# dendisuhubdy/neural_sound_generation

Hardware: AMD Instinct MI355X
Metric: mel-frames/sec VQ-VAE fwd+bwd+Adam (80-mel x 1024) (higher is better)
Workload: dtype bf16; 1 GPU; BASELINE configs[1]: VQVAE(1,dim=128,z_dim=512) train step, 128 clips/GPU x 80-mel x 1024 frames; clips_per_gpu=128, global_batch=128, frames=1024, parallelism=dp1

## Files before the change

### include/nsg.h

```cpp
#ifndef NSG_H_
#define NSG_H_

#include <stdint.h>
#include <stddef.h>

#ifdef __cplusplus
extern "C" {
#endif

#if defined(__GNUC__)
#define NSG_API __attribute__((visibility("default")))
#else
#define NSG_API
#endif

#define NSG_VERSION 104

enum {
    NSG_OK = 0,
    NSG_E_INVALID = -1,
    NSG_E_UNSUPPORTED = -2,
    NSG_E_WORKSPACE = -3
};

// ... 126 lines not shown
                            size_t workspace_bytes, void *stream);

NSG_API size_t nsg_c1conv_bn_workspace_bytes(int32_t C);
NSG_API int nsg_c1conv_bn_relu_forward(const float *img, const float *w, const float *bias, const float *gamma, const float *beta,
                                       float *mean, float *invstd, float *running_mean, float *running_var, float eps,
                                       float momentum, int32_t training, void *y, int32_t y_dtype, int32_t B, int32_t H,
                                       int32_t W, int32_t C, void *workspace, size_t workspace_bytes, double *moments,
                                       void *stream);
NSG_API int nsg_c1conv_bn_relu_backward(const float *img, const float *w, const float *bias, const float *gamma,
                                        const float *beta, const float *mean, const float *invstd, const void *dy,
                                        int32_t dy_dtype, float *dw, float *dbias, float *dgamma, float *dbeta, int32_t B,
                                        int32_t H, int32_t W, int32_t C, void *workspace, size_t workspace_bytes,
                                        const double *moments, void *stream);
#define NSG_C1_MOMENTS 273

NSG_API int32_t nsg_bn_relu_c1convt_supported(int32_t dtype, int32_t C);
NSG_API size_t nsg_bn_relu_c1convt_workspace_bytes(int32_t B, int32_t H, int32_t W, int32_t C);
NSG_API int nsg_bn_relu_c1convt_forward(const void *u, int32_t dtype, const float *mean, const float *invstd, const float *gamma,
                                        const float *beta, const float *w, const float *bias, float *y, int32_t flags, int32_t B,
                                        int32_t H, int32_t W, int32_t C, void *workspace, size_t workspace_bytes, void *stream);
NSG_API int nsg_bn_relu_c1convt_forward_mse(const void *u, int32_t dtype, const float *mean, const float *invstd, const float *gamma,
                                            const float *beta, const float *w, const float *bias, float *y, const float *target,
                                            int32_t T, float grad_scale, float *loss_out, float *dpre, float *dbias, int32_t B,
                                            int32_t H, int32_t W, int32_t C, void *workspace, size_t workspace_bytes, void *stream);
NSG_API int nsg_bn_relu_c1convt_backward(const void *u, int32_t dtype, const float *mean, const float *invstd, const float *gamma,
                                         const float *beta, const float *w, const float *dy, void *du, float *du_colsum, float *dw,
                                         float *dbias, float *dgamma, float *dbeta, int32_t B, int32_t H, int32_t W, int32_t C,
                                         void *workspace, size_t workspace_bytes, void *stream);

NSG_API int32_t nsg_bn_relu_conv1x1_supported(int32_t dtype, int32_t C);
// ... 239 lines not shown
```

### neural_sound_generation_amd/_lib.py

```python
from __future__ import annotations

import ctypes
import os
import re
from ctypes import POINTER, Structure, c_char_p, c_float, c_int32, c_int64, c_size_t, c_void_p

from .build import INCLUDE

_PKG = os.path.dirname(os.path.abspath(__file__))
LIB_PATH = os.path.join(_PKG, "libnsg.so")
HEADER_PATH = os.path.join(INCLUDE, "nsg.h")


class NsgError(RuntimeError):
    pass


class ConvDesc(Structure):

    def key(self):
        return tuple(getattr(self, f) for f, _ in self._fields_)


_SCALARS = {"int": c_int32, "int32_t": c_int32, "int64_t": c_int64, "size_t": c_size_t, "float": c_float}
# ... 50 lines not shown
            return parse_header(f.read())
    except OSError as e:
        raise NsgError(f"{HEADER_PATH}: cannot read the ABI header ({e})")


_SIGS, _CONSTS, _fields = _header()
if not _fields:
    raise NsgError(f"{HEADER_PATH}: struct nsg_conv_desc not found")
ConvDesc._fields_ = [(f, c_int32) for f in _fields]
HEADER_SYMBOLS = list(_SIGS)
NSG_VERSION = _CONSTS["NSG_VERSION"]
NSG_RELU_IN, NSG_TANH_OUT, NSG_OUT_F32, NSG_RELU_OUT, NSG_F32, NSG_BF16, NSG_C1_MOMENTS = (_CONSTS[n] for n in (
    "NSG_RELU_IN", "NSG_TANH_OUT", "NSG_OUT_F32", "NSG_RELU_OUT", "NSG_F32", "NSG_BF16", "NSG_C1_MOMENTS"))
NSG_DTW_MAX_FRAMES, NSG_DTW_BLOCK_COLS = _CONSTS["NSG_DTW_MAX_FRAMES"], _CONSTS["NSG_DTW_BLOCK_COLS"]
NSG_F0_MAX_CANDIDATES, NSG_F0_VITERBI_LDS_FRAMES = _CONSTS["NSG_F0_MAX_CANDIDATES"], _CONSTS["NSG_F0_VITERBI_LDS_FRAMES"]

_lib = None


def _bind(lib):
    for name, (res, args) in _SIGS.items():
        fn = getattr(lib, name)
        fn.argtypes = args
        fn.restype = res
    if lib.nsg_version() != NSG_VERSION:
        raise NsgError(f"the HIP library reports ABI version {lib.nsg_version()}, include/nsg.h declares version {NSG_VERSION}: rebuild it "
                       "(python -m neural_sound_generation_amd.build --force)")
    return lib


DIAG_LIB_PATH = os.path.join(_PKG, "libnsg_diag.so")
_DIAG_SWITCHES = {"nsg_debug_set_patch_gemm": c_int32, "nsg_debug_set_patch_grid": c_int32, "nsg_debug_set_wgrad_strip": c_int32,
                  "nsg_debug_set_c1_moments": c_int32, "nsg_debug_set_wgrad_bf16_native": c_int32, "nsg_debug_set_wgrad_stagger": c_int32,
                  "nsg_debug_set_wgrad_diag": c_int32, "nsg_debug_set_wgrad_stamp_buffer": c_void_p, "nsg_debug_set_stamp_buffer": c_void_p,
                  "nsg_debug_set_f0_direct": c_int32}
_diag = None


def load_diag():
    global _diag
    if _diag is None:
        import torch
        if not os.path.exists(DIAG_LIB_PATH):
            raise NsgError(f"{DIAG_LIB_PATH} is missing: python -m neural_sound_generation_amd.build --diag")
        lib = _bind(ctypes.CDLL(DIAG_LIB_PATH))
        for name, at in _DIAG_SWITCHES.items():
            fn = getattr(lib, name)
            fn.argtypes = [at]
            fn.restype = None
        _diag = lib
# ... 60 lines not shown
```

### neural_sound_generation_amd/csrc/c1_mfma.hip

```cpp
#include "nsg_reduce.h"
#include "c1_geom.h"
#include <type_traits>

namespace {

typedef float v2f __attribute__((ext_vector_type(2)));

template <int NT> struct PatchRegs { static constexpr int N = (PATCH_VALS + NT - 1) / NT; };

template <int NT>
__device__ __forceinline__ void patch_load(float (&r)[PatchRegs<NT>::N], const float *__restrict__ img, const C1Geom &g, int b, int ly, int ox0, int tid)
{
    constexpr int NCOL = 2 * TW + 2;
#pragma unroll
    for (int q = 0; q < PatchRegs<NT>::N; ++q) {
        const int i = tid + NT * q;
        const int rr = i / NCOL, cix = i - rr * NCOL;
        const int y = 2 * ly - 1 + rr, x = 2 * ox0 - 1 + cix;
        const bool ok = (i < PATCH_VALS) & (y >= 0) & (y < g.HH) & (x >= 0) & (x < g.WW);
        const float v = img[ok ? ((size_t)b * g.HH + y) * g.WW + x : 0];
        r[q] = ok ? v : 0.f;
    }
}
template <int NT>
// ... 738 lines not shown
    }
    const double bs = b + sft * wsum;
    const double Sp = mom[mom_sum(t)];
    const double St = Sp + (double)M * sft;
    const double X = is * (pw + (bs - mu) * Sp);
    const double G = (double)dw[e];
    dw[e] = (float)(sc * (G - (double)dbeta[c] * inv * St - (double)dgamma[c] * inv * X));
    if (t == 0 && dbias) {
        double sh = (double)M * bs;
#pragma unroll
        for (int u = 0; u < 16; ++u) sh += (double)w[(size_t)c * 16 + u] * mom[mom_sum(u)];
        dbias[c] = (float)(-sc * (double)dgamma[c] * inv * is * (sh - (double)M * mu));
    }
}

template <int NW>
__global__ __launch_bounds__(256) void bnrelu_dots_kernel(const bf16_t *__restrict__ u, const float *__restrict__ mean,
                                                          const float *__restrict__ invstd, const float *__restrict__ gamma,
                                                          const float *__restrict__ beta, const float *__restrict__ w,
                                                          float *__restrict__ dots, int64_t M)
{
    constexpr int C = 32 * NW, KS = C / 16, ROWS = 128, CPR = C / 8, PIECES = ROWS * CPR / 256;
    __shared__ __attribute__((aligned(16))) bf16_t tile[ROWS * gpitch(C)];
    __shared__ __attribute__((aligned(16))) float cfs[C], coff[C];
    const int tid = threadIdx.x, lane = tid & 63, wave = tid >> 6;
    const int n = lane & 31, hb = lane >> 5;
    for (int c = tid; c < C; c += 256) {
        const float fs = invstd[c] * gamma[c];
        cfs[c] = fs;
        coff[c] = __builtin_fmaf(-mean[c], fs, beta[c]);
    }
    v4u wa[KS];
#pragma unroll
    for (int ks = 0; ks < KS; ++ks)
#pragma unroll
        for (int i = 0; i < 4; ++i) {
            const int c0 = 16 * ks + 8 * hb + 2 * i;
            const unsigned pk = pack_bf16(w[(size_t)c0 * 16 + (n & 15)], w[(size_t)(c0 + 1) * 16 + (n & 15)]);
            wa[ks][i] = n < 16 ? pk : 0u;
        }
    const int64_t ntiles = (M + ROWS - 1) / ROWS;
    v4f pr[PIECES];
    auto prefetch = [&](int64_t t) {
#pragma unroll
        for (int i = 0; i < PIECES; ++i) {
            const int q = tid + 256 * i;
            const int row = q / CPR, cc = q - row * CPR;
            const int64_t m = t * ROWS + row;
            pr[i] = *reinterpret_cast<const v4f *>(u + (size_t)(m < M ? m : M - 1) * C + 8 * cc);
        }
    };
    auto stage = [&]() {
#pragma unroll
        for (int i = 0; i < PIECES; ++i) {
            const int q = tid + 256 * i;
            const int row = q / CPR, cc = q - row * CPR;
            *reinterpret_cast<v4f *>(tile + row * gpitch(C) + 8 * cc) = pr[i];
        }
    };
    if ((int64_t)blockIdx.x < ntiles) { prefetch(blockIdx.x); stage(); }
    __syncthreads();
    for (int64_t t = blockIdx.x; t < ntiles; t += gridDim.x) {
        const int64_t nxt = t + gridDim.x;
        if (nxt < ntiles) prefetch(nxt);
        v16f acc;
#pragma unroll
        for (int r = 0; r < 16; ++r) acc[r] = 0.f;
        const bf16_t *rowp = tile + (32 * wave + n) * gpitch(C) + 8 * hb;
#pragma unroll
        for (int ks = 0; ks < KS; ++ks) {
            const v4f raw = *reinterpret_cast<const v4f *>(rowp + 16 * ks);
            const v4f f0 = *reinterpret_cast<const v4f *>(cfs + 16 * ks + 8 * hb), f1 = *reinterpret_cast<const v4f *>(cfs + 16 * ks + 8 * hb + 4);
            const v4f o0 = *reinterpret_cast<const v4f *>(coff + 16 * ks + 8 * hb), o1 = *reinterpret_cast<const v4f *>(coff + 16 * ks + 8 * hb + 4);
            const float fs8[8] = {f0.x, f0.y, f0.z, f0.w, f1.x, f1.y, f1.z, f1.w};
            const float of8[8] = {o0.x, o0.y, o0.z, o0.w, o1.x, o1.y, o1.z, o1.w};
            float uv[8];
            Elem<bf16_t>::unpack16(raw, uv);
            v4u a;
#pragma unroll
            for (int i = 0; i < 4; ++i)
                a[i] = pack_bf16(fmaxf(__builtin_fmaf(uv[2 * i], fs8[2 * i], of8[2 * i]), 0.f),
                                 fmaxf(__builtin_fmaf(uv[2 * i + 1], fs8[2 * i + 1], of8[2 * i + 1]), 0.f));
            acc = __builtin_amdgcn_mfma_f32_32x32x16_bf16(__builtin_bit_cast(bf16x8, wa[ks]), __builtin_bit_cast(bf16x8, a), acc, 0, 0, 0);
        }
        const int64_t m = t * ROWS + 32 * wave + n;
        if (m < M) {
            *reinterpret_cast<v4f *>(dots + (size_t)m * 16 + 4 * hb) = v4f{acc[0], acc[1], acc[2], acc[3]};
            *reinterpret_cast<v4f *>(dots + (size_t)m * 16 + 8 + 4 * hb) = v4f{acc[4], acc[5], acc[6], acc[7]};
        }
        __syncthreads();
        if (nxt < ntiles) stage();
        __syncthreads();
    }
}

}

bool nsg_c1m_supported(int C) { return (C % 32 == 0 && C >= 32 && C <= 128) || C == 256; }

#define NSG_C1M_DISPATCH(KERNEL, ...)                                                                                   \
    switch (C / 32) {                                                                                                   \
    case 1: hipLaunchKernelGGL((KERNEL<1>), dim3(blocks), dim3(64), 0, s, __VA_ARGS__); break;                          \
    case 2: hipLaunchKernelGGL((KERNEL<2>), dim3(blocks), dim3(128), 0, s, __VA_ARGS__); break;                         \
    case 3: hipLaunchKernelGGL((KERNEL<3>), dim3(blocks), dim3(192), 0, s, __VA_ARGS__); break;                         \
    case 8: hipLaunchKernelGGL((KERNEL<8>), dim3(blocks), dim3(512), 0, s, __VA_ARGS__); break;                         \
    default: hipLaunchKernelGGL((KERNEL<4>), dim3(blocks), dim3(256), 0, s, __VA_ARGS__); break;                        \
    }
// ... 98 lines not shown
    int64_t blocks = (M + 127) / 128;
    const int64_t cap = C > 128 ? 512 : 1024;
    if (blocks > cap) blocks = cap;
    if (blocks < 1) return NSG_OK;
    const bf16_t *ub = reinterpret_cast<const bf16_t *>(u);
    switch (C / 32) {
    case 1: hipLaunchKernelGGL((bnrelu_dots_kernel<1>), dim3((unsigned)blocks), dim3(256), 0, s, ub, mean, invstd, gamma, beta, w, dots, M); break;
    case 2: hipLaunchKernelGGL((bnrelu_dots_kernel<2>), dim3((unsigned)blocks), dim3(256), 0, s, ub, mean, invstd, gamma, beta, w, dots, M); break;
    case 3: hipLaunchKernelGGL((bnrelu_dots_kernel<3>), dim3((unsigned)blocks), dim3(256), 0, s, ub, mean, invstd, gamma, beta, w, dots, M); break;
    case 8: hipLaunchKernelGGL((bnrelu_dots_kernel<8>), dim3((unsigned)blocks), dim3(256), 0, s, ub, mean, invstd, gamma, beta, w, dots, M); break;
    default: hipLaunchKernelGGL((bnrelu_dots_kernel<4>), dim3((unsigned)blocks), dim3(256), 0, s, ub, mean, invstd, gamma, beta, w, dots, M); break;
    }
    return nsg_check_launch("bnrelu_dots_kernel");
}

int nsg_launch_c1m_out_bwd_sums(const float *dimg, const float *w, const void *u, const float *mean, const float *invstd, const float *gamma,
                                const float *beta, float *partial, int blocks, int B, int LH, int LW, int C, hipStream_t s)
{
    const C1Geom g = make_geom(B, LH, LW, 2 * LH, 2 * LW, C);
    NSG_C1M_DISPATCH2(c1m_bwd_sums_kernel, true, dimg, w, (const float *)nullptr, reinterpret_cast<const bf16_t *>(u), mean, invstd, gamma, beta,
                      partial, g)
    return nsg_check_launch("c1m_bwd_sums_kernel<out>");
}

int nsg_launch_c1m_out_bwd_apply(const float *dimg, const float *w, const void *u, const float *mean, const float *invstd, const float *gamma,
                                 const float *beta, const float *dgamma, const float *dbeta, float inv_m, float *partial17, void *du, int blocks,
                                 int B, int LH, int LW, int C, hipStream_t s)
{
    const C1Geom g = make_geom(B, LH, LW, 2 * LH, 2 * LW, C);
    NSG_C1M_DISPATCH2(c1m_bwd_wgrad_kernel, true, dimg, w, (const float *)nullptr, reinterpret_cast<const bf16_t *>(u), mean, invstd, gamma, beta,
// ... 4 lines not shown
```

### neural_sound_generation_amd/csrc/conv_api.hip

```cpp
#include "nsg_reduce.h"

NSG_DIAG_SWITCH(unsigned long long *, g_debug_stamps, nullptr)
#ifdef NSG_DIAG
extern "C" NSG_API void nsg_debug_set_stamp_buffer(unsigned long long *buf) { g_debug_stamps = buf; }
#endif

namespace {

struct PackJob {
    const float *src;
    void *dst;
    int T, NN, CC, sn, sc, flip, bf16, frag;
};
constexpr int PACK_MAX_JOBS = 32;
struct PackJobs {
    PackJob job[PACK_MAX_JOBS];
};
__global__ __launch_bounds__(256) void pack_w_kernel(const PackJobs jobs)
{
    const PackJob j = jobs.job[blockIdx.y];
    const int64_t total = (int64_t)j.T * j.NN * j.CC;
    if (j.bf16 && j.CC % 8 == 0 && (reinterpret_cast<uintptr_t>(j.dst) & 15u) == 0) {
        typedef unsigned u4 __attribute__((ext_vector_type(4)));
        const int CG = j.CC / 8;
// ... 25 lines not shown
                reinterpret_cast<bf16_t *>(j.dst)[total + nsg_frag_index(t, n, c, j.NN, j.CC)] = nsg_f2bf(v);
            }
        } else {
            reinterpret_cast<float *>(j.dst)[i] = v;
        }
    }
}

constexpr int C1_COL2IM_TY = 4, C1_COL2IM_TX = 64;
inline int col2im_blocks(int B, int HH, int WW)
{
    const int64_t nt = (int64_t)B * (((HH + 1) / 2 + C1_COL2IM_TY - 1) / C1_COL2IM_TY) * (((WW + 1) / 2 + C1_COL2IM_TX - 1) / C1_COL2IM_TX);
    return (int)(nt < C1_LOSS_BLOCKS ? (nt < 1 ? 1 : nt) : C1_LOSS_BLOCKS);
}

__device__ __forceinline__ float c1_tanh(float x)
{
    const float t = __expf(-2.f * fabsf(x));
    return copysignf(__fdividef(1.f - t, 1.f + t), x);
}
constexpr int C2I_TY = C1_COL2IM_TY, C2I_TX = C1_COL2IM_TX;
static_assert(C2I_TY * C2I_TX == 256, "one thread per position");
template <bool LOSS>
__global__ __launch_bounds__(256) void col2im_c1_kernel(const float *__restrict__ dots, const float *__restrict__ bias, float *__restrict__ out,
                                                        int B, int LH, int LW, int HH, int WW, int tanh_out, const float *__restrict__ target,
                                                        int T, float gscale, float *__restrict__ dpre, double *__restrict__ partial)
{
    typedef float f2 __attribute__((ext_vector_type(2)));
    constexpr int RY = C2I_TY + 2, RX = C2I_TX + 2, RP = 16 + 4;
    __shared__ __attribute__((aligned(16))) float rec[RY * RX * RP];
    const int PY = (HH + 1) / 2, PX = (WW + 1) / 2;
    const int tiles_y = (PY + C2I_TY - 1) / C2I_TY, tiles_x = (PX + C2I_TX - 1) / C2I_TX;
    const int64_t ntiles = (int64_t)B * tiles_y * tiles_x;
    const int tid = threadIdx.x;
    const int py = tid / C2I_TX, px = tid - py * C2I_TX;
    const float bv = bias ? bias[0] : 0.f;
    const bool vec = (T & 1) == 0, vec_out = (WW & 1) == 0;
    double lacc = 0.0, gacc = 0.0;
    constexpr int NPC = (RY * RX * 4 + 255) / 256;
    v4f pc[NPC];
    auto tile_coords = [&](int64_t tile, int &b, int &ly0, int &lx0) {
        const int tx = (int)(tile % tiles_x);
        const int ty = (int)((tile / tiles_x) % tiles_y);
// ... 31 lines not shown
        if (ly >= PY || lx >= PX) continue;
        const float *rc = rec + ((py + 1) * RX + (px + 1)) * RP;
        auto tap = [&](int m, int n, int kh, int kw) { return rc[((m - 1) * RX + (n - 1)) * RP + 4 * kh + kw]; };
        float o[2][2];
        o[0][0] = (((bv + tap(1, 1, 1, 1)) + tap(1, 0, 1, 3)) + tap(0, 1, 3, 1)) + tap(0, 0, 3, 3);
        o[0][1] = (((bv + tap(1, 2, 1, 0)) + tap(1, 1, 1, 2)) + tap(0, 2, 3, 0)) + tap(0, 1, 3, 2);
        o[1][0] = (((bv + tap(2, 1, 0, 1)) + tap(2, 0, 0, 3)) + tap(1, 1, 2, 1)) + tap(1, 0, 2, 3);
        o[1][1] = (((bv + tap(2, 2, 0, 0)) + tap(2, 1, 0, 2)) + tap(1, 2, 2, 0)) + tap(1, 1, 2, 2);
        float l4 = 0.f, g4 = 0.f;
#pragma unroll
        for (int j = 0; j < 2; ++j) {
            const int yo = 2 * ly + j, xo = 2 * lx;
            if (yo >= HH) continue;
            const bool two = xo + 1 < WW;
            const size_t io = ((size_t)b * HH + yo) * WW + xo;
            const float v0 = tanh_out ? c1_tanh(o[j][0]) : o[j][0], v1 = tanh_out ? c1_tanh(o[j][1]) : o[j][1];
            if (out) {
                if (vec_out) *reinterpret_cast<f2 *>(out + io) = f2{v0, v1};
                else { out[io] = v0; if (two) out[io + 1] = v1; }
            }
            if (LOSS) {
                const float *tp = target + ((size_t)b * HH + yo) * T + xo;
                f2 tv;
                if (vec) tv = *reinterpret_cast<const f2 *>(tp);
                else { tv.x = tp[0]; tv.y = two ? tp[1] : 0.f; }
                const float d0 = v0 - tv.x, d1 = two ? v1 - tv.y : 0.f;
                l4 = __builtin_fmaf(d1, d1, __builtin_fmaf(d0, d0, l4));
                const float gp0 = gscale * d0 * (1.f - v0 * v0), gp1 = two ? gscale * d1 * (1.f - v1 * v1) : 0.f;
                if (vec_out) *reinterpret_cast<f2 *>(dpre + io) = f2{gp0, gp1};
                else { dpre[io] = gp0; if (two) dpre[io + 1] = gp1; }
                g4 += gp0;
                g4 += gp1;
                if (lx == PX - 1)
                    for (int xx = WW; xx < T; ++xx) {
                        const float cv = target[((size_t)b * HH + yo) * T + xx];
                        lacc += (double)(cv * cv);
                    }
            }
        }
        lacc += (double)l4;
        gacc += (double)g4;
    }
    if (LOSS) {
        nsg_block_sum_four_walk(lacc, partial);
        __syncthreads();
        nsg_block_sum_four_walk(gacc, partial + gridDim.x);
    }
}

constexpr int CS_MAX_SLABS = 512;
template <typename TI>
__global__ __launch_bounds__(256) void colsum_partial_kernel(const TI *__restrict__ x, int64_t M, int C, int slab_rows,
                                                             float *__restrict__ partial)
{
    __shared__ float red[256];
    const int tid = threadIdx.x;
    const int Cb = C < 256 ? C : 256;
    const int rgroups = 256 / Cb;
    const int cl = tid % Cb, rg = tid / Cb;
    const int64_t r0 = (int64_t)blockIdx.x * slab_rows;
    const int64_t r1 = min(M, r0 + slab_rows);
    for (int cb = 0; cb < C; cb += Cb) {
// ... 492 lines not shown

int nsg_bn_relu_c1convt_forward(const void *u, int32_t dtype, const float *mean, const float *invstd, const float *gamma, const float *beta,
                                const float *w, const float *bias, float *y, int32_t flags, int32_t B, int32_t H, int32_t W, int32_t C,
                                void *workspace, size_t workspace_bytes, void *stream)
{
    NSG_REQUIRE(u && mean && invstd && gamma && beta && w && y, NSG_E_INVALID, "nsg_bn_relu_c1convt_forward: null pointer");
    NSG_REQUIRE(B > 0 && H > 0 && W > 0, NSG_E_INVALID, "nsg_bn_relu_c1convt_forward: bad extent");
    NSG_REQUIRE(nsg_bn_relu_c1convt_supported(dtype, C), NSG_E_UNSUPPORTED,
                "nsg_bn_relu_c1convt_forward: needs bf16 tensors and C = 32, 64, 96 or 128 (use the separate operators otherwise)");
    NSG_REQUIRE(!(flags & ~NSG_TANH_OUT), NSG_E_UNSUPPORTED, "nsg_bn_relu_c1convt_forward: only NSG_TANH_OUT");
    NSG_REQUIRE(nsg_aligned16(u) && nsg_aligned16(w), NSG_E_INVALID, "nsg_bn_relu_c1convt_forward: u and w must be 16-byte aligned");
    NSG_REQUIRE(workspace && workspace_bytes >= nsg_bn_relu_c1convt_workspace_bytes(B, H, W, C), NSG_E_WORKSPACE,
                "nsg_bn_relu_c1convt_forward: workspace too small");
    NSG_REQUIRE((int64_t)B * H * W * C <= 0x7fffffffLL * 4, NSG_E_UNSUPPORTED, "nsg_bn_relu_c1convt_forward: tensor too large");
    hipStream_t s = (hipStream_t)stream;
    float *dots = c1t_fwd_layout(workspace, B, H, W).dots;
    int rc = nsg_launch_bnrelu_dots(u, mean, invstd, gamma, beta, w, dots, (int64_t)B * H * W, C, s);
    if (rc) return rc;
    hipLaunchKernelGGL(col2im_c1_kernel<false>, dim3(col2im_blocks(B, 2 * H, 2 * W)), dim3(256), 0, s, dots, bias, y, B, H, W, 2 * H,
                       2 * W, (flags & NSG_TANH_OUT) ? 1 : 0, (const float *)nullptr, 0, 0.f, (float *)nullptr, (double *)nullptr);
    return nsg_check_launch("col2im_c1_kernel");
}

int nsg_bn_relu_c1convt_forward_mse(const void *u, int32_t dtype, const float *mean, const float *invstd, const float *gamma, const float *beta,
                                    const float *w, const float *bias, float *y, const float *target, int32_t T, float grad_scale,
                                    float *loss_out, float *dpre, float *dbias, int32_t B, int32_t H, int32_t W, int32_t C, void *workspace,
                                    size_t workspace_bytes, void *stream)
{
    NSG_REQUIRE(u && mean && invstd && gamma && beta && w && target && loss_out && dpre, NSG_E_INVALID, "nsg_bn_relu_c1convt_forward_mse: null pointer");
    NSG_REQUIRE(B > 0 && H > 0 && W > 0 && T >= 2 * W, NSG_E_INVALID, "nsg_bn_relu_c1convt_forward_mse: bad extent (T >= 2W)");
    NSG_REQUIRE(nsg_bn_relu_c1convt_supported(dtype, C), NSG_E_UNSUPPORTED,
                "nsg_bn_relu_c1convt_forward_mse: needs bf16 tensors and C = 32, 64, 96, 128 or 256 (use the separate operators otherwise)");
    NSG_REQUIRE(nsg_aligned16(u) && nsg_aligned16(w), NSG_E_INVALID, "nsg_bn_relu_c1convt_forward_mse: u and w must be 16-byte aligned");
    NSG_REQUIRE(workspace && workspace_bytes >= nsg_bn_relu_c1convt_workspace_bytes(B, H, W, C), NSG_E_WORKSPACE,
                "nsg_bn_relu_c1convt_forward_mse: workspace too small");
    NSG_REQUIRE((int64_t)B * H * W * C <= 0x7fffffffLL * 4, NSG_E_UNSUPPORTED, "nsg_bn_relu_c1convt_forward_mse: tensor too large");
    hipStream_t s = (hipStream_t)stream;
    const C1tFwdLayout L = c1t_fwd_layout(workspace, B, H, W);
    float *dots = L.dots;
    double *partial = L.partial;
    int rc = nsg_launch_bnrelu_dots(u, mean, invstd, gamma, beta, w, dots, (int64_t)B * H * W, C, s);
    if (rc) return rc;
    const int64_t n = (int64_t)B * 2 * H * T;
    const int nb = col2im_blocks(B, 2 * H, 2 * W);
    hipLaunchKernelGGL(col2im_c1_kernel<true>, dim3(nb), dim3(256), 0, s, dots, bias, y, B, H, W, 2 * H, 2 * W, 1, target, T,
                       grad_scale * 2.0f / (float)n, dpre, partial);
    rc = nsg_check_launch("col2im_c1_kernel<loss>");
    if (rc) return rc;
    rc = nsg_launch_final_mean(partial, nb, (double)n, loss_out, s);
    if (rc || !dbias) return rc;
    return nsg_launch_final_mean(partial + nb, nb, 1.0, dbias, s);
}

int nsg_bn_relu_c1convt_backward(const void *u, int32_t dtype, const float *mean, const float *invstd, const float *gamma, const float *beta,
                                 const float *w, const float *dy, void *du, float *du_colsum, float *dw, float *dbias, float *dgamma,
                                 float *dbeta, int32_t B, int32_t H, int32_t W, int32_t C, void *workspace, size_t workspace_bytes,
                                 void *stream)
{
    NSG_REQUIRE(u && mean && invstd && gamma && beta && w && dy && du && dw && dgamma && dbeta, NSG_E_INVALID,
                "nsg_bn_relu_c1convt_backward: null pointer");
    NSG_REQUIRE(B > 0 && H > 0 && W > 0, NSG_E_INVALID, "nsg_bn_relu_c1convt_backward: bad extent");
    NSG_REQUIRE(nsg_bn_relu_c1convt_supported(dtype, C), NSG_E_UNSUPPORTED,
                "nsg_bn_relu_c1convt_backward: needs bf16 tensors and C = 32, 64, 96 or 128 (use the separate operators otherwise)");
    NSG_REQUIRE(nsg_aligned16(u) && nsg_aligned16(du) && nsg_aligned16(w), NSG_E_INVALID, "nsg_bn_relu_c1convt_backward: u, du and w must be 16-byte aligned");
    NSG_REQUIRE(workspace && workspace_bytes >= nsg_bn_relu_c1convt_workspace_bytes(B, H, W, C), NSG_E_WORKSPACE,
                "nsg_bn_relu_c1convt_backward: workspace too small");
// ... 146 lines not shown
```

### neural_sound_generation_amd/csrc/nsg_common.h

```cpp
#pragma once
#include <hip/hip_runtime.h>
#include <stdint.h>
#include <stdio.h>
#include <stdarg.h>
#include <atomic>
#include <initializer_list>
#include "nsg.h"

typedef float v4f __attribute__((ext_vector_type(4)));
typedef float v16f __attribute__((ext_vector_type(16)));
typedef short s16x8 __attribute__((ext_vector_type(8)));
typedef short s16x4 __attribute__((ext_vector_type(4)));
typedef __bf16 bf16x8 __attribute__((ext_vector_type(8)));
typedef unsigned short bf16_t;

__host__ __device__ __forceinline__ unsigned nsg_fbits(float f) { return __builtin_bit_cast(unsigned, f); }
__host__ __device__ __forceinline__ float nsg_bitsf(unsigned u) { return __builtin_bit_cast(float, u); }

__device__ __forceinline__ bf16_t nsg_f2bf(float f) { return __builtin_bit_cast(bf16_t, (__bf16)f); }
typedef float nsg_v2f __attribute__((ext_vector_type(2)));
typedef __bf16 nsg_bf16x2 __attribute__((ext_vector_type(2)));
__device__ __forceinline__ unsigned nsg_pack_bf16(float a, float b)
{
    const nsg_v2f f = {a, b};
// ... 213 lines not shown
int nsg_launch_flat1x1_backward(const void *h, const void *dy, const float *mean, const float *invstd, const float *gamma, const float *dgamma,
                                const float *dbeta, const float *w, void *dh, void *dx, int64_t M, int C, void *ws, int *nblocks,
                                const void *prev_x, const float *prev_mean, const float *prev_invstd, const float *prev_gamma,
                                const float *prev_beta, float **prev_partial, hipStream_t s);
bool nsg_flat1x1_fused_bwd_supported(int dtype, int C);
size_t nsg_flat1x1_fused_bwd_workspace_bytes(int C);
int nsg_launch_flat1x1_fused_bwd(const void *h, const void *dy, const float *mean, const float *invstd, const float *gamma, const float *dgamma,
                                 const float *dbeta, const float *w, void *dx, float *dw, int64_t M, int C, void *ws, int *nblocks,
                                 const void *prev_x, const float *prev_mean, const float *prev_invstd, const float *prev_gamma,
                                 const float *prev_beta, float **colsum_partial, float **prev_partial, float **dw_partial, hipStream_t s);
int nsg_launch_final_mean(const double *partial, int n, double denom, float *out, hipStream_t s);
constexpr int C1_LOSS_BLOCKS = 1024;
bool nsg_c1m_supported(int C);
int nsg_launch_bnrelu_dots(const void *u, const float *mean, const float *invstd, const float *gamma, const float *beta, const float *w,
                           float *dots, int64_t M, int C, hipStream_t s);
int nsg_launch_c1m_out_bwd_sums(const float *dimg, const float *w, const void *u, const float *mean, const float *invstd, const float *gamma,
                                const float *beta, float *partial, int blocks, int B, int LH, int LW, int C, hipStream_t s);
int nsg_launch_c1m_out_bwd_apply(const float *dimg, const float *w, const void *u, const float *mean, const float *invstd, const float *gamma,
                                 const float *beta, const float *dgamma, const float *dbeta, float inv_m, float *partial17, void *du, int blocks,
                                 int B, int LH, int LW, int C, hipStream_t s);
int nsg_launch_c1m_stats(const float *img, const float *w, const float *bias, float *tiles, int blocks, int B, int LH, int LW, int HH, int WW,
                         int C, hipStream_t s);
int nsg_launch_c1m_apply(const float *img, const float *w, const float *bias, const float *mean, const float *invstd, const float *gamma,
                         const float *beta, void *out, int blocks, int B, int LH, int LW, int HH, int WW, int C, hipStream_t s);
int nsg_launch_c1m_bwd_sums(const float *img, const float *w, const float *bias, const void *dy, const float *mean, const float *invstd,
                            const float *gamma, const float *beta, float *partial, int blocks, int B, int LH, int LW, int HH, int WW, int C,
                            hipStream_t s);
int nsg_launch_c1m_bwd_wgrad(const float *img, const float *w, const float *bias, const void *dy, const float *mean, const float *invstd,
                             const float *gamma, const float *beta, const float *dgamma, const float *dbeta, float inv_m, float *partial,
                             int blocks, int B, int LH, int LW, int HH, int WW, int C, hipStream_t s);
// ... 15 lines not shown
```

Measured before the change: 16.82 million mel-frames/s.

## Fuse BN-ReLU dots and col2im into banded transposed-conv kernel

Adds a banded kernel for the final transposed conv that computes the BN+ReLU 1x1 dot products with MFMA per row band and resolves the col2im overlap in shared memory. It emits tanh output, the MSE loss and dpre directly, so the intermediate dots tensor no longer makes a round trip through global memory. The two final-mean launches are also merged into one two-block kernel. In exchange the new kernel has halo recomputation, more synchronisation per row, and a more complex loss and boundary path.

New measurement: 16.92 million mel-frames/s, median of 6. Within noise of the previous version (+0.6%).

```diff
diff --git a/include/nsg.h b/include/nsg.h
--- a/include/nsg.h
+++ b/include/nsg.h
@@ -164,6 +164,8 @@
                                         const double *moments, void *stream);
 #define NSG_C1_MOMENTS 273
 
+#define NSG_C1T_BAND_COLS 128
+#define NSG_C1T_BAND_ROWS 64
 NSG_API int32_t nsg_bn_relu_c1convt_supported(int32_t dtype, int32_t C);
 NSG_API size_t nsg_bn_relu_c1convt_workspace_bytes(int32_t B, int32_t H, int32_t W, int32_t C);
 NSG_API int nsg_bn_relu_c1convt_forward(const void *u, int32_t dtype, const float *mean, const float *invstd, const float *gamma,
diff --git a/neural_sound_generation_amd/_lib.py b/neural_sound_generation_amd/_lib.py
--- a/neural_sound_generation_amd/_lib.py
+++ b/neural_sound_generation_amd/_lib.py
@@ -88,6 +88,7 @@
     "NSG_RELU_IN", "NSG_TANH_OUT", "NSG_OUT_F32", "NSG_RELU_OUT", "NSG_F32", "NSG_BF16", "NSG_C1_MOMENTS"))
 NSG_DTW_MAX_FRAMES, NSG_DTW_BLOCK_COLS = _CONSTS["NSG_DTW_MAX_FRAMES"], _CONSTS["NSG_DTW_BLOCK_COLS"]
 NSG_F0_MAX_CANDIDATES, NSG_F0_VITERBI_LDS_FRAMES = _CONSTS["NSG_F0_MAX_CANDIDATES"], _CONSTS["NSG_F0_VITERBI_LDS_FRAMES"]
+NSG_C1T_BAND_COLS, NSG_C1T_BAND_ROWS = _CONSTS["NSG_C1T_BAND_COLS"], _CONSTS["NSG_C1T_BAND_ROWS"]
 
 _lib = None
 
@@ -107,7 +108,7 @@
 _DIAG_SWITCHES = {"nsg_debug_set_patch_gemm": c_int32, "nsg_debug_set_patch_grid": c_int32, "nsg_debug_set_wgrad_strip": c_int32,
                   "nsg_debug_set_c1_moments": c_int32, "nsg_debug_set_wgrad_bf16_native": c_int32, "nsg_debug_set_wgrad_stagger": c_int32,
                   "nsg_debug_set_wgrad_diag": c_int32, "nsg_debug_set_wgrad_stamp_buffer": c_void_p, "nsg_debug_set_stamp_buffer": c_void_p,
-                  "nsg_debug_set_f0_direct": c_int32}
+                  "nsg_debug_set_f0_direct": c_int32, "nsg_debug_set_c1t_banded": c_int32}
 _diag = None
 
 
diff --git a/neural_sound_generation_amd/csrc/c1_emit.h b/neural_sound_generation_amd/csrc/c1_emit.h
--- /dev/null
+++ b/neural_sound_generation_amd/csrc/c1_emit.h
@@ -0,0 +1,38 @@
+#pragma once
+#include "nsg_common.h"
+
+typedef float c1_f2 __attribute__((ext_vector_type(2)));
+
+__device__ __forceinline__ float c1_tanh(float x)
+{
+    const float t = __expf(-2.f * fabsf(x));
+    return copysignf(__fdividef(1.f - t, 1.f + t), x);
+}
+
+__device__ __forceinline__ c1_f2 c1_target_pair(const float *__restrict__ tp, bool vec, bool two)
+{
+    c1_f2 tv;
+    if (vec) tv = *reinterpret_cast<const c1_f2 *>(tp);
+    else { tv.x = tp[0]; tv.y = two ? tp[1] : 0.f; }
+    return tv;
+}
+
+template <bool LOSS>
+__device__ __forceinline__ void c1_emit_pair(float o0, float o1, int tanh_out, float *__restrict__ out, size_t io, bool vec_out, bool two,
+                                             c1_f2 tv, float gscale, float *__restrict__ dpre, float &l4, float &g4)
+{
+    const float v0 = tanh_out ? c1_tanh(o0) : o0, v1 = tanh_out ? c1_tanh(o1) : o1;
+    if (out) {
+        if (vec_out) *reinterpret_cast<c1_f2 *>(out + io) = c1_f2{v0, v1};
+        else { out[io] = v0; if (two) out[io + 1] = v1; }
+    }
+    if (LOSS) {
+        const float d0 = v0 - tv.x, d1 = two ? v1 - tv.y : 0.f;
+        l4 = __builtin_fmaf(d1, d1, __builtin_fmaf(d0, d0, l4));
+        const float gp0 = gscale * d0 * (1.f - v0 * v0), gp1 = two ? gscale * d1 * (1.f - v1 * v1) : 0.f;
+        if (vec_out) *reinterpret_cast<c1_f2 *>(dpre + io) = c1_f2{gp0, gp1};
+        else { dpre[io] = gp0; if (two) dpre[io + 1] = gp1; }
+        g4 += gp0;
+        g4 += gp1;
+    }
+}
diff --git a/neural_sound_generation_amd/csrc/c1_mfma.hip b/neural_sound_generation_amd/csrc/c1_mfma.hip
--- a/neural_sound_generation_amd/csrc/c1_mfma.hip
+++ b/neural_sound_generation_amd/csrc/c1_mfma.hip
@@ -1,5 +1,6 @@
 #include "nsg_reduce.h"
 #include "c1_geom.h"
+#include "c1_emit.h"
 #include <type_traits>
 
 namespace {
@@ -776,6 +777,44 @@
     }
 }
 
+template <int KS>
+__device__ __forceinline__ void dots_w_operand(const float *__restrict__ w, int n, int hb, v4u (&wa)[KS])
+{
+#pragma unroll
+    for (int ks = 0; ks < KS; ++ks)
+#pragma unroll
+        for (int i = 0; i < 4; ++i) {
+            const int c0 = 16 * ks + 8 * hb + 2 * i;
+            const unsigned pk = pack_bf16(w[(size_t)c0 * 16 + (n & 15)], w[(size_t)(c0 + 1) * 16 + (n & 15)]);
+            wa[ks][i] = n < 16 ? pk : 0u;
+        }
+}
+template <int KS>
+__device__ __forceinline__ v16f dots_block(const bf16_t *row, const float *cfs, const float *coff, int hb, const v4u (&wa)[KS])
+{
+    v16f acc;
+#pragma unroll
+    for (int r = 0; r < 16; ++r) acc[r] = 0.f;
+    const bf16_t *rowp = row + 8 * hb;
+#pragma unroll
+    for (int ks = 0; ks < KS; ++ks) {
+        const v4f raw = *reinterpret_cast<const v4f *>(rowp + 16 * ks);
+        const v4f f0 = *reinterpret_cast<const v4f *>(cfs + 16 * ks + 8 * hb), f1 = *reinterpret_cast<const v4f *>(cfs + 16 * ks + 8 * hb + 4);
+        const v4f o0 = *reinterpret_cast<const v4f *>(coff + 16 * ks + 8 * hb), o1 = *reinterpret_cast<const v4f *>(coff + 16 * ks + 8 * hb + 4);
+        const float fs8[8] = {f0.x, f0.y, f0.z, f0.w, f1.x, f1.y, f1.z, f1.w};
+        const float of8[8] = {o0.x, o0.y, o0.z, o0.w, o1.x, o1.y, o1.z, o1.w};
+        float uv[8];
+        Elem<bf16_t>::unpack16(raw, uv);
+        v4u a;
+#pragma unroll
+        for (int i = 0; i < 4; ++i)
+            a[i] = pack_bf16(fmaxf(__builtin_fmaf(uv[2 * i], fs8[2 * i], of8[2 * i]), 0.f),
+                             fmaxf(__builtin_fmaf(uv[2 * i + 1], fs8[2 * i + 1], of8[2 * i + 1]), 0.f));
+        acc = __builtin_amdgcn_mfma_f32_32x32x16_bf16(__builtin_bit_cast(bf16x8, wa[ks]), __builtin_bit_cast(bf16x8, a), acc, 0, 0, 0);
+    }
+    return acc;
+}
+
 template <int NW>
 __global__ __launch_bounds__(256) void bnrelu_dots_kernel(const bf16_t *__restrict__ u, const float *__restrict__ mean,
                                                           const float *__restrict__ invstd, const float *__restrict__ gamma,
@@ -793,14 +832,7 @@
         coff[c] = __builtin_fmaf(-mean[c], fs, beta[c]);
     }
     v4u wa[KS];
-#pragma unroll
-    for (int ks = 0; ks < KS; ++ks)
-#pragma unroll
-        for (int i = 0; i < 4; ++i) {
-            const int c0 = 16 * ks + 8 * hb + 2 * i;
-            const unsigned pk = pack_bf16(w[(size_t)c0 * 16 + (n & 15)], w[(size_t)(c0 + 1) * 16 + (n & 15)]);
-            wa[ks][i] = n < 16 ? pk : 0u;
-        }
+    dots_w_operand<KS>(w, n, hb, wa);
     const int64_t ntiles = (M + ROWS - 1) / ROWS;
     v4f pr[PIECES];
     auto prefetch = [&](int64_t t) {
@@ -825,26 +857,7 @@
     for (int64_t t = blockIdx.x; t < ntiles; t += gridDim.x) {
         const int64_t nxt = t + gridDim.x;
         if (nxt < ntiles) prefetch(nxt);
-        v16f acc;
-#pragma unroll
-        for (int r = 0; r < 16; ++r) acc[r] = 0.f;
-        const bf16_t *rowp = tile + (32 * wave + n) * gpitch(C) + 8 * hb;
-#pragma unroll
-        for (int ks = 0; ks < KS; ++ks) {
-            const v4f raw = *reinterpret_cast<const v4f *>(rowp + 16 * ks);
-            const v4f f0 = *reinterpret_cast<const v4f *>(cfs + 16 * ks + 8 * hb), f1 = *reinterpret_cast<const v4f *>(cfs + 16 * ks + 8 * hb + 4);
-            const v4f o0 = *reinterpret_cast<const v4f *>(coff + 16 * ks + 8 * hb), o1 = *reinterpret_cast<const v4f *>(coff + 16 * ks + 8 * hb + 4);
-            const float fs8[8] = {f0.x, f0.y, f0.z, f0.w, f1.x, f1.y, f1.z, f1.w};
-            const float of8[8] = {o0.x, o0.y, o0.z, o0.w, o1.x, o1.y, o1.z, o1.w};
-            float uv[8];
-            Elem<bf16_t>::unpack16(raw, uv);
-            v4u a;
-#pragma unroll
-            for (int i = 0; i < 4; ++i)
-                a[i] = pack_bf16(fmaxf(__builtin_fmaf(uv[2 * i], fs8[2 * i], of8[2 * i]), 0.f),
-                                 fmaxf(__builtin_fmaf(uv[2 * i + 1], fs8[2 * i + 1], of8[2 * i + 1]), 0.f));
-            acc = __builtin_amdgcn_mfma_f32_32x32x16_bf16(__builtin_bit_cast(bf16x8, wa[ks]), __builtin_bit_cast(bf16x8, a), acc, 0, 0, 0);
-        }
+        const v16f acc = dots_block<KS>(tile + (32 * wave + n) * gpitch(C), cfs, coff, hb, wa);
         const int64_t m = t * ROWS + 32 * wave + n;
         if (m < M) {
             *reinterpret_cast<v4f *>(dots + (size_t)m * 16 + 4 * hb) = v4f{acc[0], acc[1], acc[2], acc[3]};
@@ -853,6 +866,137 @@
         __syncthreads();
         if (nxt < ntiles) stage();
         __syncthreads();
+    }
+}
+
+constexpr int BC = NSG_C1T_BAND_COLS, BREC = BC + 2, BTP = BREC + 2;
+static_assert(BC == 128, "c1t_banded_kernel: four waves of 32 records + the halo pair; 2 x 128 emitting threads");
+template <int NW, bool LOSS>
+__global__ __launch_bounds__(256) __attribute__((amdgpu_waves_per_eu(2))) void c1t_banded_kernel(const bf16_t *__restrict__ u, const float *__restrict__ mean,
+                                                         const float *__restrict__ invstd, const float *__restrict__ gamma,
+                                                         const float *__restrict__ beta, const float *__restrict__ w,
+                                                         const float *__restrict__ bias, float *__restrict__ out, int B, int H, int W,
+                                                         int band_rows, int tanh_out, const float *__restrict__ target, int T, float gscale,
+                                                         float *__restrict__ dpre, double *__restrict__ partial)
+{
+    constexpr int C = 32 * NW, KS = C / 16, CPR = C / 8, NPIECE = BREC * CPR, PIECES = (NPIECE + 255) / 256;
+    __shared__ __attribute__((aligned(16))) bf16_t tile[BREC * gpitch(C)];
+    __shared__ __attribute__((aligned(16))) float cfs[C], coff[C];
+    __shared__ float lo[8 * BTP], hi[2][8 * BTP];
+    const int tid = threadIdx.x, lane = tid & 63, wave = tid >> 6;
+    const int n = lane & 31, hb = lane >> 5;
+    const int ej = tid >> 7, elx = tid & (BC - 1);
+    for (int c = tid; c < C; c += 256) {
+        const float fs = invstd[c] * gamma[c];
+        cfs[c] = fs;
+        coff[c] = __builtin_fmaf(-mean[c], fs, beta[c]);
+    }
+    v4u wa[KS];
+    dots_w_operand<KS>(w, n, hb, wa);
+    const float bv = bias ? bias[0] : 0.f;
+    const int HH = 2 * H, WW = 2 * W;
+    const bool vec = (T & 1) == 0;
+    const int nby = (H + band_rows - 1) / band_rows, nbx = (W + BC - 1) / BC;
+    const int64_t nbands = (int64_t)B * nby * nbx;
+    double lacc = 0.0, gacc = 0.0;
+
+    for (int64_t band = blockIdx.x; band < nbands; band += gridDim.x) {
+        const int bx = (int)(band % nbx), by = (int)((band / nbx) % nby), b = (int)(band / ((int64_t)nbx * nby));
+        const int x0 = bx * BC, y0 = by * band_rows, y1 = min(H, y0 + band_rows);
+        const int ys = y0 > 0 ? y0 - 1 : 0;
+        const int ye = y1 == H ? H : y1 - 1;
+        const int vb = min(ye, H - 1);
+
+        unsigned poff[PIECES];
+#pragma unroll
+        for (int i = 0; i < PIECES; ++i) {
+            const int q = tid + 256 * i;
+            const int rec = min(q / CPR, BREC - 1), cc = q % CPR;
+            poff[i] = (unsigned)min(max(x0 - 1 + rec, 0), W - 1) * C + 8 * cc;
+        }
+        const int elxc = min(x0 + elx, W - 1);
+        const unsigned dead = 8u * (tid & 15);
+        auto fetch = [&](v4f (&pr)[PIECES], c1_f2 &tg, int yy) {
+            const bool live = yy <= vb;
+            const bf16_t *rowp = u + ((size_t)b * H + min(yy, vb)) * W * C;
+#pragma unroll
+            for (int i = 0; i < PIECES; ++i) pr[i] = *reinterpret_cast<const v4f *>(rowp + (live ? poff[i] : min(poff[i], dead)));
+            if (LOSS) {
+                const int yo = min(max(2 * min(yy, ye) - 1 + ej, 0), HH - 1);
+                tg = c1_target_pair(target + ((size_t)b * HH + yo) * T + 2 * (yy <= ye ? elxc : min(elxc, tid & 15)), vec, true);
+            }
+        };
+        auto park = [&](int rec, int y, const v16f &acc) {
+            const int col = x0 - 1 + rec;
+            const bool ok = col >= 0 && col < W;
+#pragma unroll
+            for (int k = 0; k < 4; ++k) {
+                lo[(4 * hb + k) * BTP + rec] = ok ? acc[k] : 0.f;
+                hi[y & 1][(4 * hb + k) * BTP + rec] = ok ? acc[4 + k] : 0.f;
+            }
+        };
+        auto step = [&](v4f (&pr)[PIECES], c1_f2 &tg, int y) {
+            const bool data = y <= vb;
+            if (data) {
+#pragma unroll
+                for (int i = 0; i < PIECES; ++i) {
+                    const int q = tid + 256 * i;
+                    if (q < NPIECE) *reinterpret_cast<v4f *>(tile + (q / CPR) * gpitch(C) + 8 * (q % CPR)) = pr[i];
+                }
+            }
+            const c1_f2 tcur = tg;
+            __syncthreads();
+            fetch(pr, tg, y + 2);
+            if (data) {
+                int z0 = 0, z1 = 0;
+                asm volatile("" : "+s"(z0), "+s"(z1));
+                const int rec = 32 * wave + n;
+                park(rec, y, dots_block<KS>(tile + rec * gpitch(C), cfs + z0, coff + z0, hb, wa));
+                if (__builtin_amdgcn_readfirstlane(wave) == (y & 3)) {
+                    const int rh = BC + n;
+                    const v16f acc = dots_block<KS>(tile + min(rh, BREC - 1) * gpitch(C), cfs + z1, coff + z1, hb, wa);
+                    if (rh < BREC) park(rh, y, acc);
+                }
+            } else {
+                for (int i = tid; i < 8 * BTP; i += 256) lo[i] = 0.f;
+            }
+            __syncthreads();
+            const int yo = 2 * y - 1 + ej;
+            const bool ok = y >= y0 && y <= ye && yo >= 0 && yo < HH && x0 + elx < W;
+            const float *cur = lo + 4 * ej * BTP + elx + 1, *prv = hi[(y & 1) ^ 1] + 4 * ej * BTP + elx + 1;
+            const float o0 = (((bv + cur[1 * BTP]) + cur[3 * BTP - 1]) + prv[1 * BTP]) + prv[3 * BTP - 1];
+            const float o1 = (((bv + cur[0 * BTP + 1]) + cur[2 * BTP]) + prv[0 * BTP + 1]) + prv[2 * BTP];
+            if (ok) {
+                float l2 = 0.f, g2 = 0.f;
+                c1_emit_pair<LOSS>(o0, o1, tanh_out, out, ((size_t)b * HH + yo) * WW + 2 * elxc, true, true, tcur, gscale, dpre, l2, g2);
+                if (LOSS) {
+                    lacc += (double)l2;
+                    gacc += (double)g2;
+                    if (elxc == W - 1)
+                        for (int xx = WW; xx < T; ++xx) {
+                            const float cv = target[((size_t)b * HH + yo) * T + xx];
+                            lacc += (double)(cv * cv);
+                        }
+                }
+            }
+        };
+
+        __syncthreads();
+        if (y0 == 0)
+            for (int i = tid; i < 8 * BTP; i += 256) hi[1][i] = 0.f;
+        v4f pa[PIECES], pb[PIECES];
+        c1_f2 ta = {0.f, 0.f}, tb = {0.f, 0.f};
+        fetch(pa, ta, ys);
+        fetch(pb, tb, ys + 1);
+        for (int y = ys; y <= ye; y += 2) {
+            step(pa, ta, y);
+            step(pb, tb, y + 1);
+        }
+    }
+    if (LOSS) {
+        nsg_block_sum_four_walk(lacc, partial);
+        __syncthreads();
+        nsg_block_sum_four_walk(gacc, partial + gridDim.x);
     }
 }
 
@@ -981,6 +1125,32 @@
     return nsg_check_launch("bnrelu_dots_kernel");
 }
 
+bool nsg_c1t_banded_supported(int C, int W) { return C % 32 == 0 && C >= 32 && C <= 128 && (int64_t)W * C < (1LL << 31); }
+
+int nsg_launch_c1t_banded(const void *u, const float *mean, const float *invstd, const float *gamma, const float *beta, const float *w,
+                          const float *bias, float *out, int B, int H, int W, int C, int band_rows, int tanh_out, const float *target, int T,
+                          float gscale, float *dpre, double *partial, int *nblocks, hipStream_t s)
+{
+    const int64_t nbands = (int64_t)B * nsg_cdiv(H, band_rows) * nsg_cdiv(W, BC);
+    const unsigned blocks = (unsigned)(nbands < C1_LOSS_BLOCKS ? nbands : C1_LOSS_BLOCKS);
+    if (nblocks) *nblocks = (int)blocks;
+    const bf16_t *ub = reinterpret_cast<const bf16_t *>(u);
+#define NSG_C1T_LAUNCH(NW)                                                                                                          \
+    if (target) hipLaunchKernelGGL((c1t_banded_kernel<NW, true>), dim3(blocks), dim3(256), 0, s, ub, mean, invstd, gamma, beta, w, bias, \
+                                   out, B, H, W, band_rows, tanh_out, target, T, gscale, dpre, partial);                            \
+    else hipLaunchKernelGGL((c1t_banded_kernel<NW, false>), dim3(blocks), dim3(256), 0, s, ub, mean, invstd, gamma, beta, w, bias, out, \
+                            B, H, W, band_rows, tanh_out, target, T, gscale, dpre, partial);                                        \
+    break;
+    switch (C / 32) {
+    case 1: NSG_C1T_LAUNCH(1)
+    case 2: NSG_C1T_LAUNCH(2)
+    case 3: NSG_C1T_LAUNCH(3)
+    default: NSG_C1T_LAUNCH(4)
+    }
+#undef NSG_C1T_LAUNCH
+    return nsg_check_launch("c1t_banded_kernel");
+}
+
 int nsg_launch_c1m_out_bwd_sums(const float *dimg, const float *w, const void *u, const float *mean, const float *invstd, const float *gamma,
                                 const float *beta, float *partial, int blocks, int B, int LH, int LW, int C, hipStream_t s)
 {
diff --git a/neural_sound_generation_amd/csrc/conv_api.hip b/neural_sound_generation_amd/csrc/conv_api.hip
--- a/neural_sound_generation_amd/csrc/conv_api.hip
+++ b/neural_sound_generation_amd/csrc/conv_api.hip
@@ -1,8 +1,11 @@
 #include "nsg_reduce.h"
+#include "c1_emit.h"
 
 NSG_DIAG_SWITCH(unsigned long long *, g_debug_stamps, nullptr)
+NSG_DIAG_SWITCH(int, g_c1t_banded, 1)
 #ifdef NSG_DIAG
 extern "C" NSG_API void nsg_debug_set_stamp_buffer(unsigned long long *buf) { g_debug_stamps = buf; }
+extern "C" NSG_API void nsg_debug_set_c1t_banded(int on) { g_c1t_banded = on; }
 #endif
 
 namespace {
@@ -63,11 +66,6 @@
     return (int)(nt < C1_LOSS_BLOCKS ? (nt < 1 ? 1 : nt) : C1_LOSS_BLOCKS);
 }
 
-__device__ __forceinline__ float c1_tanh(float x)
-{
-    const float t = __expf(-2.f * fabsf(x));
-    return copysignf(__fdividef(1.f - t, 1.f + t), x);
-}
 constexpr int C2I_TY = C1_COL2IM_TY, C2I_TX = C1_COL2IM_TX;
 static_assert(C2I_TY * C2I_TX == 256, "one thread per position");
 template <bool LOSS>
@@ -75,7 +73,6 @@
                                                         int B, int LH, int LW, int HH, int WW, int tanh_out, const float *__restrict__ target,
                                                         int T, float gscale, float *__restrict__ dpre, double *__restrict__ partial)
 {
-    typedef float f2 __attribute__((ext_vector_type(2)));
     constexpr int RY = C2I_TY + 2, RX = C2I_TX + 2, RP = 16 + 4;
     __shared__ __attribute__((aligned(16))) float rec[RY * RX * RP];
     const int PY = (HH + 1) / 2, PX = (WW + 1) / 2;
@@ -137,29 +134,14 @@
             if (yo >= HH) continue;
             const bool two = xo + 1 < WW;
             const size_t io = ((size_t)b * HH + yo) * WW + xo;
-            const float v0 = tanh_out ? c1_tanh(o[j][0]) : o[j][0], v1 = tanh_out ? c1_tanh(o[j][1]) : o[j][1];
-            if (out) {
-                if (vec_out) *reinterpret_cast<f2 *>(out + io) = f2{v0, v1};
-                else { out[io] = v0; if (two) out[io + 1] = v1; }
-            }
-            if (LOSS) {
-                const float *tp = target + ((size_t)b * HH + yo) * T + xo;
-                f2 tv;
-                if (vec) tv = *reinterpret_cast<const f2 *>(tp);
-                else { tv.x = tp[0]; tv.y = two ? tp[1] : 0.f; }
-                const float d0 = v0 - tv.x, d1 = two ? v1 - tv.y : 0.f;
-                l4 = __builtin_fmaf(d1, d1, __builtin_fmaf(d0, d0, l4));
-                const float gp0 = gscale * d0 * (1.f - v0 * v0), gp1 = two ? gscale * d1 * (1.f - v1 * v1) : 0.f;
-                if (vec_out) *reinterpret_cast<f2 *>(dpre + io) = f2{gp0, gp1};
-                else { dpre[io] = gp0; if (two) dpre[io + 1] = gp1; }
-                g4 += gp0;
-                g4 += gp1;
-                if (lx == PX - 1)
-                    for (int xx = WW; xx < T; ++xx) {
-                        const float cv = target[((size_t)b * HH + yo) * T + xx];
-                        lacc += (double)(cv * cv);
-                    }
-            }
+            c1_f2 tv = {0.f, 0.f};
+            if (LOSS) tv = c1_target_pair(target + ((size_t)b * HH + yo) * T + xo, vec, two);
+            c1_emit_pair<LOSS>(o[j][0], o[j][1], tanh_out, out, io, vec_out, two, tv, gscale, dpre, l4, g4);
+            if (LOSS && lx == PX - 1)
+                for (int xx = WW; xx < T; ++xx) {
+                    const float cv = target[((size_t)b * HH + yo) * T + xx];
+                    lacc += (double)(cv * cv);
+                }
         }
         lacc += (double)l4;
         gacc += (double)g4;
@@ -169,6 +151,16 @@
         __syncthreads();
         nsg_block_sum_four_walk(gacc, partial + gridDim.x);
     }
+}
+
+__global__ __launch_bounds__(64) void c1t_final_kernel(const double *__restrict__ partial, int n, double denom, float *__restrict__ loss_out,
+                                                       float *__restrict__ dbias)
+{
+    const bool second = blockIdx.x == 1;
+    nsg_wave_close_sum(partial + (second ? n : 0), n, [&](double s) {
+        if (second) dbias[0] = (float)s;
+        else loss_out[0] = (float)(s / denom);
+    });
 }
 
 constexpr int CS_MAX_SLABS = 512;
@@ -691,6 +683,9 @@
                 "nsg_bn_relu_c1convt_forward: workspace too small");
     NSG_REQUIRE((int64_t)B * H * W * C <= 0x7fffffffLL * 4, NSG_E_UNSUPPORTED, "nsg_bn_relu_c1convt_forward: tensor too large");
     hipStream_t s = (hipStream_t)stream;
+    if (g_c1t_banded && nsg_c1t_banded_supported(C, W))
+        return nsg_launch_c1t_banded(u, mean, invstd, gamma, beta, w, bias, y, B, H, W, C, NSG_C1T_BAND_ROWS, (flags & NSG_TANH_OUT) ? 1 : 0,
+                                     nullptr, 0, 0.f, nullptr, nullptr, nullptr, s);
     float *dots = c1t_fwd_layout(workspace, B, H, W).dots;
     int rc = nsg_launch_bnrelu_dots(u, mean, invstd, gamma, beta, w, dots, (int64_t)B * H * W, C, s);
     if (rc) return rc;
@@ -714,19 +709,25 @@
     NSG_REQUIRE((int64_t)B * H * W * C <= 0x7fffffffLL * 4, NSG_E_UNSUPPORTED, "nsg_bn_relu_c1convt_forward_mse: tensor too large");
     hipStream_t s = (hipStream_t)stream;
     const C1tFwdLayout L = c1t_fwd_layout(workspace, B, H, W);
-    float *dots = L.dots;
     double *partial = L.partial;
-    int rc = nsg_launch_bnrelu_dots(u, mean, invstd, gamma, beta, w, dots, (int64_t)B * H * W, C, s);
-    if (rc) return rc;
     const int64_t n = (int64_t)B * 2 * H * T;
-    const int nb = col2im_blocks(B, 2 * H, 2 * W);
-    hipLaunchKernelGGL(col2im_c1_kernel<true>, dim3(nb), dim3(256), 0, s, dots, bias, y, B, H, W, 2 * H, 2 * W, 1, target, T,
-                       grad_scale * 2.0f / (float)n, dpre, partial);
-    rc = nsg_check_launch("col2im_c1_kernel<loss>");
-    if (rc) return rc;
-    rc = nsg_launch_final_mean(partial, nb, (double)n, loss_out, s);
-    if (rc || !dbias) return rc;
-    return nsg_launch_final_mean(partial + nb, nb, 1.0, dbias, s);
+    const float gscale = grad_scale * 2.0f / (float)n;
+    int rc, nb;
+    if (g_c1t_banded && nsg_c1t_banded_supported(C, W)) {
+        rc = nsg_launch_c1t_banded(u, mean, invstd, gamma, beta, w, bias, y, B, H, W, C, NSG_C1T_BAND_ROWS, 1, target, T, gscale, dpre, partial,
+                                   &nb, s);
+        if (rc) return rc;
+    } else {
+        rc = nsg_launch_bnrelu_dots(u, mean, invstd, gamma, beta, w, L.dots, (int64_t)B * H * W, C, s);
+        if (rc) return rc;
+        nb = col2im_blocks(B, 2 * H, 2 * W);
+        hipLaunchKernelGGL(col2im_c1_kernel<true>, dim3(nb), dim3(256), 0, s, L.dots, bias, y, B, H, W, 2 * H, 2 * W, 1, target, T, gscale, dpre,
+                           partial);
+        rc = nsg_check_launch("col2im_c1_kernel<loss>");
+        if (rc) return rc;
+    }
+    hipLaunchKernelGGL(c1t_final_kernel, dim3(dbias ? 2 : 1), dim3(64), 0, s, partial, nb, (double)n, loss_out, dbias);
+    return nsg_check_launch("c1t_final_kernel");
 }
 
 int nsg_bn_relu_c1convt_backward(const void *u, int32_t dtype, const float *mean, const float *invstd, const float *gamma, const float *beta,
diff --git a/neural_sound_generation_amd/csrc/nsg_common.h b/neural_sound_generation_amd/csrc/nsg_common.h
--- a/neural_sound_generation_amd/csrc/nsg_common.h
+++ b/neural_sound_generation_amd/csrc/nsg_common.h
@@ -251,6 +251,10 @@
 bool nsg_c1m_supported(int C);
 int nsg_launch_bnrelu_dots(const void *u, const float *mean, const float *invstd, const float *gamma, const float *beta, const float *w,
                            float *dots, int64_t M, int C, hipStream_t s);
+bool nsg_c1t_banded_supported(int C, int W);
+int nsg_launch_c1t_banded(const void *u, const float *mean, const float *invstd, const float *gamma, const float *beta, const float *w,
+                          const float *bias, float *out, int B, int H, int W, int C, int band_rows, int tanh_out, const float *target, int T,
+                          float gscale, float *dpre, double *partial, int *nblocks, hipStream_t s);
 int nsg_launch_c1m_out_bwd_sums(const float *dimg, const float *w, const void *u, const float *mean, const float *invstd, const float *gamma,
                                 const float *beta, float *partial, int blocks, int B, int LH, int LW, int C, hipStream_t s);
 int nsg_launch_c1m_out_bwd_apply(const float *dimg, const float *w, const void *u, const float *mean, const float *invstd, const float *gamma,
```
